# uzh-rpg/dagr

Measured on AMD Instinct MI355X. Metric: events_per_sec, higher is better.
Workload: dtype f32; 1 GPU; dagr-s + --use_image --img_net resnet50, 640x480 synthetic S-uniform, B=8 windows/step x 100000 events (50 ms each), r=7, K=16, events->graph->GNN(+image fusion)->decoded head outputs->confidence mask + NMS (device); image_branch=in-line, engines=3

## Files before the change

dagr_amd/engine.py:

```python
import contextlib
import ctypes
import gc
import types

import numpy as np
import torch

from . import _lib
from .graph.ev_graph import WindowGraphBuilder

FUSED_PASSES_MAX_NODES = 1600

L0_WIDTHS = (8, 16, 32)


def _l0_block(c):
    cm = max(b for b in (0,) + L0_WIDTHS if b <= c)
    return cm, c - cm


def _f32(v):
    return float(torch.as_tensor(v, dtype=torch.float32))


# ... 16 lines not shown
    with torch.cuda.graph(graph):
        gc.disable()
        try:
            yield
        finally:
            if was_enabled:
                gc.enable()

class _ConvPack:

    def __init__(self, cin, cskip, Wm, bias, relu):
        self.K, self.N = Wm.shape
        self.ldw = (self.N + 7) // 8 * 8
        if self.ldw != self.N:
            Wm = torch.cat([Wm, torch.zeros((self.K, self.ldw - self.N), dtype=Wm.dtype, device=Wm.device)], 1)
        self.cin, self.cskip, self.Wm, self.bias, self.relu = cin, cskip, Wm.contiguous(), bias.contiguous(), relu
        K16, N16 = (self.K + 15) // 16 * 16, (self.N + 15) // 16 * 16
        Wp = torch.zeros((K16, N16), dtype=Wm.dtype, device=Wm.device)
        Wp[: self.K, : self.N] = Wm[:, : self.N]
        self.Wq = Wp.view(K16 // 16, 4, 4, N16 // 16, 16).permute(3, 0, 2, 4, 1).contiguous()


def _pack_generic(convs, norms, skip=None, relu=True, device="cuda"):
    cols, biases = [], []
    cin = convs[0].in_channels
    for conv, norm in zip(convs, norms):
        W = conv.weight.detach().float()
        root = conv.lin.weight.detach().float()
        cout = W.shape[2]
        if norm is not None:
            scale, shift = _bn_affine(norm)
        else:
            scale, shift = torch.ones(cout, device=W.device), torch.zeros(cout, device=W.device)
        if conv.bias is not None:
            shift = shift + conv.bias.detach().float() * scale
        block = torch.cat([W.reshape(25 * cin, cout), root.t()], 0) * scale.view(1, -1)
        if skip is not None:
            lin, norm_skip = skip
            s_scale, s_shift = _bn_affine(norm_skip)
            block = torch.cat([block, lin.mlp.weight.detach().float().t() * s_scale.view(1, -1)], 0)
            shift = shift + s_shift
        cols.append(block)
        biases.append(shift)
    cskip = skip[0].mlp.in_features if skip is not None else 0
    return _ConvPack(cin, cskip, torch.cat(cols, 1).to(device), torch.cat(biases).to(device), relu)


def _pack_l0(conv, norm, win, skip=None, device="cuda", cols_in=None, cols_skip=None):
    win_x, tx, win_y, ty = win
    W = conv.weight.detach().float()
    cin, cout = W.shape[1], W.shape[2]
    if cout not in L0_WIDTHS:
        raise NotImplementedError(f"the level-0 kernels exist for {', '.join(map(str, L0_WIDTHS))} output channels "
                                  f"(base_width = 0.25, 0.5, 1.0), not {cout}")
    cols_in = list(range(cin)) if cols_in is None else list(cols_in)
    scale, shift = _bn_affine(norm)
    rows = []
    for b in range(ty):
        for a in range(tx):
            rows.append(W[(win_x + a) + 5 * (win_y + b)][cols_in] * scale.view(1, -1))
    rows.append(conv.lin.weight.detach().float().t()[cols_in] * scale.view(1, -1))
    cskip = 0
    if skip is not None:
        lin, norm_skip = skip
        s_scale, s_shift = _bn_affine(norm_skip)
        ws = lin.mlp.weight.detach().float().t()
        if cols_skip is not None:
            ws = ws[list(cols_skip)]
        rows.append(ws * s_scale.view(1, -1))
        shift = shift + s_shift
        cskip = lin.mlp.in_features
    return cin, cskip, torch.cat(rows, 0).contiguous().to(device), shift.contiguous().to(device)


class _Conv1x1Gemm(torch.nn.Module):

    def __init__(self, conv, relu=False):
        super().__init__()
        cout, cin = conv.weight.shape[:2]
        self.stride = conv.stride[0]
        self.relu = relu
        self.register_buffer("wt", conv.weight.detach().reshape(cout, cin).t().contiguous())
        self.register_buffer("b", conv.bias.detach().clone() if conv.bias is not None else torch.zeros(cout, device=conv.weight.device))

    def forward(self, x, residual=None):
        if self.stride != 1:
            x = x[:, :, ::self.stride, ::self.stride]
        B, C, H, W = x.shape
        a = x.permute(0, 2, 3, 1).reshape(-1, C)
        N = self.wt.shape[1]
        r = None if residual is None else residual.permute(0, 2, 3, 1)
        if _LT["ok"] and a.is_cuda and a.dtype == torch.float32 and a.stride(1) == 1 \
                and (r is None or (r.is_contiguous() and tuple(r.shape) == (B, H, W, N))):
            y = torch.empty((a.shape[0], N), dtype=torch.float32, device=a.device)
            ws = _lt_workspace(a.device)
            act = 1 if (self.relu or r is not None) else 0
            rc = _lib.lib().dagr_gemm_epilogue(_lib.ptr(a), a.shape[0], C, a.stride(0), _lib.ptr(self.wt), N,
                                               _lib.ptr(self.b), _lib.ptr(r), N, act, _lib.ptr(y), N, _lib.ptr(ws),
                                               ws.numel(), _lib.cur_stream(a.device))
            if rc == 0:
                return y.view(B, H, W, -1).permute(0, 3, 1, 2)
            _LT["ok"] = False
        if residual is not None:
            y = torch.addmm(self.b, a, self.wt).view(B, H, W, -1).permute(0, 3, 1, 2)
            return _add_relu_(y, residual)
        y = torch._addmm_activation(self.b, a, self.wt) if self.relu else torch.addmm(self.b, a, self.wt)
        return y.view(B, H, W, -1).permute(0, 3, 1, 2)


_LT = {"ok": True, "ws": {}}


def _lt_workspace(device):
    key = str(device)
    if key not in _LT["ws"]:
        _LT["ws"][key] = torch.empty(int(_lib.lib().dagr_gemm_epilogue_workspace_bytes()), dtype=torch.uint8, device=device)
    return _LT["ws"][key]


def _gemmify_1x1(module):
    for name, child in list(module.named_children()):
        if isinstance(child, torch.nn.Conv2d) and child.kernel_size == (1, 1) and child.groups == 1 \
                and child.padding == (0, 0) and child.stride[0] == child.stride[1]:
            setattr(module, name, _Conv1x1Gemm(child))
        else:
            _gemmify_1x1(child)


def _add_relu_(y, z):
    if y.is_cuda and y.dtype == torch.float32 and z.dtype == torch.float32 and y.shape == z.shape \
            and y.stride() == z.stride() and y.data_ptr() % 16 == 0 and z.data_ptr() % 16 == 0 \
            and (y.is_contiguous() or y.is_contiguous(memory_format=torch.channels_last)):
        _lib.check(_lib.lib().dagr_add_relu(_lib.ptr(y), _lib.ptr(z), y.numel(), _lib.cur_stream(y.device)), "add_relu")
        return y
    return torch.relu_(y.add_(z))


def _bias_relu_(y, bias):
    C = y.shape[1]
    if y.is_cuda and y.dtype == torch.float32 and C % 4 == 0 and y.is_contiguous(memory_format=torch.channels_last) \
            and y.data_ptr() % 16 == 0 and bias.data_ptr() % 16 == 0:
        _lib.check(_lib.lib().dagr_bias_relu(_lib.ptr(y), _lib.ptr(bias), y.numel(), C, _lib.cur_stream(y.device)),
                   "bias_relu")
        return y
    return torch.relu_(y.add_(bias.view(1, -1, 1, 1)))


def _baseconv_forward(m, x):
    y = m.conv(x)
    b = m._bias
    C = y.shape[1]
    if y.is_cuda and y.dtype == torch.float32 and C % 4 == 0 and y.is_contiguous(memory_format=torch.channels_last) \
            and y.data_ptr() % 16 == 0 and b.data_ptr() % 16 == 0:
        _lib.check(_lib.lib().dagr_bias_silu(_lib.ptr(y), _lib.ptr(b), y.numel(), C, _lib.cur_stream(y.device)),
                   "bias_silu")
        return y
    return torch.nn.functional.silu(y.add_(b.view(1, -1, 1, 1)), inplace=True)


def _conv_bias_relu(blk, name, x):
    conv = getattr(blk, name)
    b = getattr(blk, "_" + name + "_bias", None)
    out = conv(x)
    if b is not None:
        return _bias_relu_(out, b)
    if getattr(conv, "relu", False):
        return out
    return blk.relu(out)


def _bottleneck_forward(blk, x):
    identity = x if blk.downsample is None else blk.downsample(x)
    out = _conv_bias_relu(blk, "conv1", x)
    out = _conv_bias_relu(blk, "conv2", out)
    if isinstance(blk.conv3, _Conv1x1Gemm):
        return blk.conv3(out, residual=identity)
    return _add_relu_(blk.conv3(out), identity)


def _resnet_features_forward(net, x, emit=None):
    emit = emit or (lambda name, t: None)
    c1 = net.conv1(x)
    emit("conv1", c1)
    mp = net.maxpool
    ok = (c1.is_cuda and c1.dtype == torch.float32 and c1.is_contiguous(memory_format=torch.channels_last)
          and c1.shape[1] % 4 == 0 and mp.kernel_size == 3 and mp.stride == 2 and mp.padding == 1
          and mp.dilation == 1 and not mp.ceil_mode)
    if ok:
        B, C, H, W = c1.shape
        scale, shift = net._stem_affine
        y = torch.empty((B, C, (H - 1) // 2 + 1, (W - 1) // 2 + 1), dtype=c1.dtype, device=c1.device,
                        memory_format=torch.channels_last)
        _lib.check(_lib.lib().dagr_bn_relu_maxpool(_lib.ptr(c1), B, H, W, C, _lib.ptr(scale), _lib.ptr(shift), _lib.ptr(y),
                                                   _lib.cur_stream(c1.device)), "bn_relu_maxpool")
    else:
        y = net.maxpool(net.relu(net.bn1(c1)))
    l1 = net.layer1(y)
    emit("layer1", l1)
    l2 = net.layer2(l1)
    emit("layer2", l2)
    l3 = net.layer3(l2)
    emit("layer3", l3)
    l4 = net.layer4(l3)
    emit("layer4", l4)
    return dict(conv1=c1, layer1=l1, layer2=l2, layer3=l3, layer4=l4)


def _basicblock_forward(blk, x):
    identity = x if blk.downsample is None else blk.downsample(x)
    out = _conv_bias_relu(blk, "conv1", x)
    return _add_relu_(blk.conv2(out), identity)


class StreamState:

    def __init__(self, batch_size, window_us, device):
        self.B, self.window_us, self.device = int(batch_size), int(window_us), torch.device(device)
        self.cap = 0
        self.state = None
        self.status = torch.zeros((1,), dtype=torch.int32, device=self.device)
        self.lane_count = torch.zeros((self.B,), dtype=torch.int32, device=self.device)
        self.image = None
        self._host = torch.zeros((self.B,), dtype=torch.int32).pin_memory()
        self._known = np.zeros((self.B,), np.int64)
        self._since = 0
        self._fresh = True

    def _alloc(self, cap):
        L = _lib.lib()
        nbytes = L.dagr_stream_state_bytes(self.B, cap)
        if nbytes == 0:
            raise RuntimeError(f"dagr_stream_state_bytes({self.B}, {cap}): out of range")
        return torch.empty(nbytes, dtype=torch.uint8, device=self.device)

    def reset(self):
        if self.state is not None:
            _lib.check(_lib.lib().dagr_stream_reset(_lib.ptr(self.state), self.B, self.cap, _lib.cur_stream(self.device)),
                       "stream_reset")
        self.status.zero_()
        self.lane_count.zero_()
        torch.cuda.current_stream(self.device).synchronize()
        self._host.zero_()
        self._known, self._since, self._fresh = np.zeros((self.B,), np.int64), 0, True

    def grow(self, cap):
# ... 432 lines not shown
                                                1 if pack.relu else 0, stream), "spline_conv_fused")
            return
        lda = (pack.K + 3) // 4 * 4
        _lib.check(L.dagr_spline_tap_aggregate(P(lvl.counts), lvl.T, P(lvl.rowptr), P(lvl.col), P(code),
                                               x, ldx, pack.cin, xskip, ldskip, pack.cskip, dom["rx"], dom["ry"],
                                               dom["den_x"], dom["den_y"], P(scratch), lda, stream), "tap_aggregate")
        _lib.check(L.dagr_gemm_bias_act(P(lvl.counts), lvl.T, P(scratch), lda, P(pack.Wm), pack.ldw, P(pack.bias),
                                        out, ldo, pack.K, pack.N, 1 if pack.relu else 0, stream), "gemm")

    def stage_graph(self, pos, batch, feat=None):
        N = int(pos.shape[0])
        self._alloc_events(N)
        self._N = N
        self._pos, self._batch = pos, batch
        self._nbr = (self.nbr_src[:N], self.nbr_code[:N], self.deg[:N])
        inputs = None
        if feat is not None and pos.dtype == torch.float32:
            self._feat_flat = feat.float().reshape(-1).contiguous()
            inputs = _lib.L0Inputs(feat=self._feat_flat.data_ptr(), pos_nodes=self.pos_n.data_ptr(),
                                   batch_nodes=self.batch_n.data_ptr(), x0=self.x0buf.data_ptr(), ldx0=self.x0_ld,
                                   col_feat=self.x0_feat_col, col_pos=self.x0_pos_col)
        self.graph.build(pos, batch, out=self._nbr, n_dev=self.n_dev if self._dev_mode else None, inputs=inputs)
        self._inputs_gathered = inputs is not None
        self._n_rows = N
        self._async_on = False

    def _nptr(self):
        return self.graph.node_count_ptr() if self._dev_mode else None

    def _sample(self, n_ptr, n_max, pos, batch, b64, fmap, out, coff):
        if self._feat_ready is not None:
            ready = self._feat_ready.get(id(fmap))
            if ready is None:
                raise RuntimeError("pipelined window: a sampled feature map has no ready-event (the image branch did not "
                                   "announce it) -- reading it would race with the image stream")
            torch.cuda.current_stream(self.device).wait_event(ready)
        Bf, C, h, w = fmap.shape
        nhwc = fmap.permute(0, 2, 3, 1)
        if not nhwc.is_contiguous():
            nhwc = nhwc.contiguous()
        self._keep.append(nhwc)
        _lib.check(self.L.dagr_sample_features(n_ptr, n_max, _lib.ptr(pos), _lib.ptr(batch), b64, _lib.ptr(nhwc), Bf, h,
                                               w, C, self.W, self.H, _lib.ptr(out), out.shape[1], coff,
                                               _lib.cur_stream(self.device)), "sample_features")

    def _fold_image_branch(self):
        import copy
        from torch.nn.utils.fusion import fuse_conv_bn_eval
        bb, head = self.model.backbone, self.model.head
        net = copy.deepcopy(bb.net).eval()
        cnn = copy.deepcopy(head.cnn_head).eval()

        def fold_block(blk):
            for ci, bi in (("conv1", "bn1"), ("conv2", "bn2"), ("conv3", "bn3")):
                if hasattr(blk, ci):
                    setattr(blk, ci, fuse_conv_bn_eval(getattr(blk, ci), getattr(blk, bi)))
                    setattr(blk, bi, torch.nn.Identity())
            if blk.downsample is not None:
                blk.downsample = torch.nn.Sequential(fuse_conv_bn_eval(blk.downsample[0], blk.downsample[1]))
        for name in ("layer1", "layer2", "layer3", "layer4"):
            for blk in getattr(net.module, name):
                fold_block(blk)
        for m in cnn.modules():
            if hasattr(m, "conv") and hasattr(m, "bn") and isinstance(m.bn, torch.nn.BatchNorm2d):
                m.conv = fuse_conv_bn_eval(m.conv, m.bn)
                m.bn = torch.nn.Identity()
                if isinstance(getattr(m, "act", None), torch.nn.SiLU) and m.conv.bias is not None:
                    m._bias = m.conv.bias.detach().clone().contiguous()
                    m.conv.bias = None
                    m.forward = types.MethodType(_baseconv_forward, m)
        net = net.to(memory_format=torch.channels_last)
        cnn = cnn.to(memory_format=torch.channels_last)
        for blkname in ("layer1", "layer2", "layer3", "layer4"):
            _gemmify_1x1(getattr(net.module, blkname))
            for blk in getattr(net.module, blkname):
                relu_convs = ("conv1", "conv2") if hasattr(blk, "conv3") else ("conv1",)
                for cname in relu_convs:
                    conv = getattr(blk, cname)
                    if isinstance(conv, _Conv1x1Gemm):
                        conv.relu = True
                    elif isinstance(conv, torch.nn.Conv2d) and conv.bias is not None:
                        setattr(blk, "_" + cname + "_bias", conv.bias.detach().clone().contiguous())
                        conv.bias = None
                blk.forward = types.MethodType(_bottleneck_forward if hasattr(blk, "conv3") else _basicblock_forward,
                                               blk)
        bn = net.module.bn1
        scale = (bn.weight.detach().float() / torch.sqrt(bn.running_var.detach().float() + bn.eps)).contiguous()
        shift = (bn.bias.detach().float() - bn.running_mean.detach().float() * scale).contiguous()
        net.module._stem_affine = (scale, shift)
        net.module.forward_features = types.MethodType(_resnet_features_forward, net.module)
        _gemmify_1x1(net.feature_dconv)
        _gemmify_1x1(net.output_dconv)
        self._net_f, self._cnn_f = net, cnn

    def _image_branch(self, image, on_feature=None):
        if self._net_f is None:
            self._fold_image_branch()
        bb, head = types.SimpleNamespace(net=self._net_f), types.SimpleNamespace(cnn_head=self._cnn_f)
        x = image.contiguous(memory_format=torch.channels_last)
        net = self._net_f
        if on_feature is not None:
            feats = [None] * len(net.feature_layers)

            def emit(name, t):
                if name in net.feature_layers:
                    j = net.feature_layers.index(name)
                    feats[j] = net.feature_dconv[j](t) if len(net.feature_dconv) > 0 else t
                    on_feature(j, feats[j])
            d = _resnet_features_forward(net.module, x, emit)
            outs = [d[l] for l in net.output_layers]
            if len(net.output_dconv) > 0:
                outs = [dconv(o) for o, dconv in zip(outs, net.output_dconv)]
        else:
            feats, outs = bb.net(x)
        outs = outs[-self.num_scales:]
        resized = [torch.nn.functional.interpolate(f, o) for f, o in zip(outs, self.out_sizes)]
        return feats, head.cnn_head(resized)

    def stage_image(self, image):
        self._keep = []
        self._img_feats, self._cnn_out = self._image_branch(image)

    def image_async(self, image, stream=None):
        cur = torch.cuda.current_stream(self.device)
        if stream is not None:
            self._img_stream = stream
        if self._img_stream is None:
            self._img_stream = torch.cuda.Stream(self.device)
        s = self._img_stream
        s.wait_stream(cur)
        with torch.cuda.stream(s):
            feats, cnn_out = self._image_branch(image)
            ev = torch.cuda.Event()
            ev.record(s)
        return feats, cnn_out, ev

    def _consume_image_handle(self, handle):
        feats, cnn_out, ev = handle
        cur = torch.cuda.current_stream(self.device)
        cur.wait_event(ev)
        for t in list(feats) + [o for v in cnn_out.values() for o in v]:
            t.record_stream(cur)
        self._keep = []
        self._img_feats, self._cnn_out = feats, cnn_out

    def stage_l0_input(self, feat):
        N = self._N
        x0 = self.x0buf[:N]
        g = self.graph
        if not self._inputs_gathered:
            f = feat.float().reshape(-1).contiguous()
            _lib.check(self.L.dagr_graph_gather_inputs(ctypes.byref(g.desc), _lib.ptr(g.workspace), _lib.ptr(self._pos),
                                                       _lib.ptr(f), N, _lib.ptr(self.pos_n), _lib.ptr(self.batch_n),
                                                       _lib.ptr(x0), self.x0_ld, self.x0_feat_col, self.x0_pos_col,
                                                       _lib.cur_stream(self.device)), "graph_gather_inputs")
        if self.use_image:
            self._sample(self._nptr(), N, self.pos_n, self.batch_n, 0, self._img_feats[0], x0, self.x0_img_col)
        self._x0 = x0

    def _conv_l0(self, pack, x, ldx, xskip, ldskip, out, ldo):
        L, P = self.L, _lib.ptr
        nbr_src, nbr_code, deg = self._nbr
        cin, cskip, w, s = pack
        d0 = self.dom[0]
        wx, tx, wy, ty = self.win0
        stream = _lib.cur_stream(self.device)
        if self.l0_tiles:
            cm, ce = self._l0_blocks[cin]
            _lib.check(L.dagr_spline_conv_l0_tiles_w(self.cout0, cm, ce, cskip, wx, tx, wy, ty, d0["rx"], d0["ry"],
                                                     d0["den_x"], d0["den_y"], self._N, self.graph.K, P(nbr_src), P(nbr_code),
                                                     P(deg), x, ldx, xskip, ldskip, P(w), P(s), 1, out, ldo, self._nptr(),
                                                     stream), "conv_l0_tiles")
        else:
            _lib.check(L.dagr_spline_conv_l0(cin, cskip, self.ntaps0, self._N, self.graph.K, self.ncodes0, P(nbr_src),
                                             P(nbr_code), P(deg), x, ldx, xskip, ldskip, P(self.tab0), P(w), P(s), 1,
                                             out, ldo, stream), "conv_l0")
# ... 581 lines not shown
```

include/dagr_hip.h:

```cpp
#ifndef DAGR_HIP_H
#define DAGR_HIP_H

#include <stddef.h>
#include <stdint.h>

#ifdef __cplusplus
extern "C" {
#endif

typedef enum {
    DAGR_OK = 0,
    DAGR_ERR_INVALID_ARG = -1,
    DAGR_ERR_HIP = -2,
    DAGR_ERR_WORKSPACE = -3,
    DAGR_ERR_UNSUPPORTED = -4
} dagr_status;

const char *dagr_last_error(void);
int dagr_version(void);
int dagr_device_count(void);

int dagr_format_events(const int16_t *xy , const int32_t *t , const int8_t *p ,
                       int64_t N, int32_t width, int32_t height, int32_t time_window,
                       float *pos_out , float *feat_out , void *stream);
// ... 216 lines not shown
int dagr_spline_conv_fused_pool(const int32_t *n_nodes_ptr, int32_t n_nodes_max, const int32_t *rowptr,
                                const int32_t *col, const int32_t *code, const float *x, int32_t ldx, int32_t cin,
                                const float *xskip, int32_t ldskip, int32_t cskip, int32_t rx, int32_t ry,
                                float den_x, float den_y, const float *Wq, const float *bias, float *C,
                                int32_t ldc, int32_t N, int32_t relu, const dagr_pool_desc *pdesc, void *pool_ws,
                                const float *pos, const int32_t *batch, int32_t *cluster_scratch, void *stream);
int dagr_pool_csr(const dagr_pool_desc *desc, void *pool_ws, const int32_t *n_ptr, int32_t n_max, const float *x,
                  int32_t ldx, const float *pos, const int32_t *batch, const int32_t *rowptr, const int32_t *col,
                  int32_t *cluster_scratch , float *x_out, int32_t ldo, int32_t xoff, float *pos_out,
                  int32_t *batch_out, int32_t *n_out, int32_t *rowptr_out, int32_t *col_out, int32_t *code_out,
                  int32_t *e_out, int32_t e_cap, void *stream);
int dagr_pool_recode(const int32_t *n_ptr, int32_t n_max, const int32_t *rowptr, const int32_t *col, const float *pos,
                     float two_max, float r00, float r02, float r11, float r12, int32_t rx, int32_t ry,
                     int32_t *code_out, int32_t e_cap, int32_t *status, void *stream);
int dagr_pool_status(const dagr_pool_desc *desc, void *pool_ws, int32_t *flags_host, void *stream);
const int32_t *dagr_pool_status_ptr(const dagr_pool_desc *desc, void *pool_ws);
int dagr_pool_counters(const dagr_pool_desc *desc, void *pool_ws, int32_t *out8_host, void *stream);

int dagr_to_dense(const int32_t *n_ptr, int32_t n_max, const float *x, int32_t ldx, int32_t channels,
                  const float *pos, const int32_t *batch, float vx, float vy, int32_t batch_size,
                  int32_t Hc, int32_t Wc, int32_t *winner_scratch, float *dense, int32_t *status, void *stream);

int dagr_pool_argmax(const int32_t *cluster, int32_t n, const float *x, int32_t ldx, int32_t channels,
                     const float *x_pooled, int32_t ldp, int32_t n_clusters, int32_t *arg, void *stream);
int dagr_pool_grad(const int32_t *cluster, int32_t n, int32_t channels, int32_t aggr, const int32_t *arg,
                   const int32_t *count, const float *grad_pooled, int32_t ldg, float *grad_x, int32_t ldgx,
                   void *stream);
int dagr_to_dense_grad(int32_t n, int32_t channels, const float *pos, const int32_t *batch, float vx, float vy,
                       int32_t batch_size, int32_t Hc, int32_t Wc, const float *grad_dense,
                       float *grad_x, int32_t ldgx, void *stream);

int dagr_add_relu(float *y, const float *z, int64_t n, void *stream);
int dagr_bias_relu(float *y_nhwc, const float *bias, int64_t n, int32_t C, void *stream);
int dagr_bias_silu(float *y_nhwc, const float *bias, int64_t n, int32_t C, void *stream);
int dagr_bn_relu_maxpool(const float *x_nhwc, int32_t B, int32_t H, int32_t W, int32_t C, const float *scale,
                         const float *shift, float *y_nhwc, void *stream);

int dagr_sample_features(const int32_t *n_ptr, int32_t n_max, const float *pos, const void *batch,
                         int32_t batch_is_int64, const float *feat_nhwc, int32_t B, int32_t h, int32_t w, int32_t C,
                         int32_t width, int32_t height, float *out, int32_t ldo, int32_t coff, void *stream);

int dagr_nms_batched(const float *boxes, const float *scores, const int32_t *cls, const uint8_t *valid,
                     int32_t B, int32_t A, float iou_threshold, float class_offset,
                     int32_t *order_out, int32_t *keep_out, int32_t *n_keep, void *stream);

typedef struct dagr_head_scale {
    const int32_t *n_ptr; int32_t n_max;
    const float *pred; int32_t ld;
    const float *pos; const int32_t *batch;
    float vx, vy, stride; int32_t Hc, Wc;
    const float *cnn[3]; int32_t cnn_stride[3][4];
    float *dense;
} dagr_head_scale;
int dagr_heads_finish(const dagr_head_scale *scale0, const dagr_head_scale *scale1, int32_t batch_size, int32_t channels,
                      float *out, int32_t *status, void *stream);
int dagr_heads_finish_detect(const dagr_head_scale *scale0, const dagr_head_scale *scale1, int32_t batch_size,
                             int32_t channels, float *out, int32_t *status, float conf_threshold, float iou_threshold,
                             float class_offset, float *det, int32_t *n_keep, void *stream);
int dagr_decode_heads(const float *dense0, int32_t H0, int32_t W0, float stride0, const float *dense1, int32_t H1,
                      int32_t W1, float stride1, int32_t B, int32_t channels, float *out, void *stream);

int dagr_postprocess(const float *pred, int32_t B, int32_t A, int32_t num_classes, float conf_threshold,
                     float iou_threshold, float class_offset, float *det, int32_t *n_keep, void *stream);

int dagr_masked_lin(const int64_t *indices, const float *x_in, float *x_out, const float *weight, const float *bias,
                    int32_t add, int64_t K, int32_t Cin, int32_t Cout, void *stream);
int dagr_masked_lin_no_bias(const int64_t *indices, const float *x_in, float *x_out, const float *weight, int32_t add,
                            int64_t K, int32_t Cin, int32_t Cout, void *stream);
int dagr_masked_isdiff(int64_t *indices, const float *x_old, const float *x_new, float atol, float rtol, int64_t K,
                       int32_t C, void *stream);
int dagr_masked_inplace_BN(const int64_t *indices, const float *x, float *x_out, const float *running_mean,
                           const float *running_var, const float *weight, const float *bias, float eps, int64_t K,
                           int32_t C, void *stream);

int dagr_downsample_events(const int32_t *order, const int32_t *run_cell, const int32_t *run_end, int32_t n_runs,
                           const int8_t *polarity, int32_t fx, int32_t fy, float *change_map, uint8_t *keep,
                           void *stream);

size_t dagr_gemm_epilogue_workspace_bytes(void);
int dagr_gemm_epilogue(const float *A, int64_t M, int32_t K, int64_t lda, const float *Wt, int32_t N, const float *bias,
                       const float *R, int64_t ldr, int32_t act, float *D, int64_t ldd, void *workspace,
                       size_t workspace_bytes, void *stream);

enum { DAGR_FLOPS_ZERO = 0, DAGR_FLOPS_CONV = 1, DAGR_FLOPS_LINEAR = 2, DAGR_FLOPS_POOL = 3, DAGR_FLOPS_CARTESIAN = 4 };
typedef struct dagr_flops_module {
    int32_t kind, level, cin, cout, root, bias;
} dagr_flops_module;
int dagr_async_flops(const int32_t *deg, int32_t n_events, const int32_t *counts1, const int32_t *counts2,
                     const int32_t *counts3, const int32_t *counts4, const dagr_flops_module *mods, int32_t n_mods,
                     int64_t *out, void *stream);

size_t dagr_viz_workspace_bytes(int32_t F, int32_t H, int32_t W);
int dagr_viz_render(const uint8_t *images, int32_t n_images, int32_t H, int32_t W, const int32_t *frame_image, int32_t F,
                    const int32_t *ev_x, const int32_t *ev_y, const int8_t *ev_p, const int32_t *ev_ptr, int32_t n_events,
                    const double *alpha, const int32_t *boxes, const int32_t *box_ptr, int32_t n_boxes, int32_t linewidth,
                    const uint8_t *colors, int32_t n_colors, uint8_t *out, int32_t *status, void *workspace,
                    size_t workspace_bytes, void *stream);

typedef struct dagr_aug_params {
    int32_t flip, crop_on;
    int32_t crop_lo[2], crop_hi[2];
    float zoom;
    int32_t move[2];
} dagr_aug_params;
size_t dagr_augment_workspace_bytes(int64_t N);
int dagr_augment_events(const dagr_aug_params *params, int32_t B, int32_t W, int32_t H, const void *pos, int32_t pos_width,
                        const void *t, int32_t t_width, const void *p, int32_t p_width, const int32_t *sample_ptr, int64_t N,
                        int16_t *out_pos, void *out_t, void *out_p, int64_t *out_batch, int32_t *out_ptr,
                        int32_t *status, void *workspace, size_t workspace_bytes, void *stream);
int dagr_augment_status(const int32_t *status, void *stream);
int dagr_augment_frames(const dagr_aug_params *params, int32_t B, int32_t C, int32_t H, int32_t W, int32_t elem_bytes,
                        int32_t reference_crop, const void *in, void *out, void *stream);
int dagr_augment_boxes(const dagr_aug_params *params, int32_t B, int32_t W, int32_t H, const float *boxes,
                       const int64_t *box_batch, int32_t M, int32_t ld, float *out, void *stream);

#define DAGR_COCO_MAX_GT 256
#define DAGR_COCO_MAX_DT 4096
#define DAGR_COCO_MAX_DETS 100
void dagr_coco_match_bounds(int32_t *max_gt, int32_t *max_dt, int32_t *max_dets);
int dagr_coco_match(const double *gt_xywh, const double *dt_xywh, const double *dt_score, const int64_t *jobs,
                    const double *area_rng, const double *iou_thrs, int32_t n_thr, int32_t max_dets, int64_t n_jobs,
                    int64_t n_gt, int64_t n_dt, int32_t max_gt_per_job, int32_t max_dt_per_job, int64_t n_out,
                    int64_t n_gign, int32_t *order, uint8_t *dtm, uint8_t *dt_ign, uint8_t *g_ign, int32_t *status,
                    void *stream);

#define DAGR_COCO_ACC_TILE 1024
#define DAGR_COCO_ACC_MAX_REC 128
int32_t dagr_coco_accumulate_tile(void);
size_t dagr_coco_accumulate_workspace_bytes(int32_t n_thr, int64_t n_cols);
int dagr_coco_accumulate(const uint8_t *dtm, const uint8_t *dt_ign, const int32_t *perm, const int64_t *group_ptr,
                         const int64_t *group_ngt, const double *rec_thrs, int32_t n_rec, double eps, int32_t n_thr,
                         int32_t n_groups, int64_t n_cols, void *workspace, size_t workspace_bytes, double *precision,
                         int32_t *status, void *stream);

int dagr_spiral_offsets(int32_t n, int32_t *dx_host, int32_t *dy_host);

#ifdef __cplusplus
}
#endif
#endif
```

Before: 143.8 million events/s.

## Route ResNet 1x1 and 3x3 convs through split-bf16 MFMA GEMM kernels

Adds a HIP GEMM kernel that splits FP32 operands into three bf16 parts and accumulates six MFMA cross products, emulating FP32 precision on the bf16 matrix units. The kernel has an implicit-im2col 3x3 mode and a strided 1x1 mode with fused bias, residual and ReLU epilogues. Weights are packed once at fold time, and size heuristics select the new path for the ResNet50 image-branch convolutions. The aim is higher matrix throughput than the FP32 library GEMM and conv paths, at the cost of extra operand splitting work and accuracy that is close to, but not exactly, FP32.

```diff
diff --git a/dagr_amd/csrc/gemm_split_bf16.hip b/dagr_amd/csrc/gemm_split_bf16.hip
--- /dev/null
+++ b/dagr_amd/csrc/gemm_split_bf16.hip
@@ -0,0 +1,334 @@
+#include <algorithm>
+
+#include "common.hpp"
+
+namespace dagr {
+namespace {
+
+constexpr int kKT = 32;
+constexpr int kBN = 128;
+constexpr int kPitch = 40;
+
+typedef __bf16 bf16x8 __attribute__((ext_vector_type(8)));
+typedef float f32x4 __attribute__((ext_vector_type(4)));
+typedef unsigned u32x4 __attribute__((ext_vector_type(4)));
+typedef unsigned u32x2 __attribute__((ext_vector_type(2)));
+
+struct Geo {
+    int mode;
+    int H, W, C, s, Ho, Wo;
+};
+
+struct Args {
+    const float *A;
+    const unsigned short *Wp;
+    const float *bias, *R;
+    float *D;
+    int64_t M, lda, ldr, ldd;
+    int K, N, Npad, act, n_tiles_n, n_blocks;
+    Geo g;
+};
+
+__device__ __forceinline__ unsigned short bf16_bits(__bf16 v) { return __builtin_bit_cast(unsigned short, v); }
+
+__device__ __forceinline__ void split3(float a, unsigned short &p1, unsigned short &p2, unsigned short &p3) {
+    const __bf16 b1 = (__bf16)a;
+    const float r1 = a - (float)b1;
+    const __bf16 b2 = (__bf16)r1;
+    const float r2 = r1 - (float)b2;
+    const __bf16 b3 = (__bf16)r2;
+    p1 = bf16_bits(b1);
+    p2 = bf16_bits(b2);
+    p3 = bf16_bits(b3);
+}
+
+__global__ __launch_bounds__(256) void k_split_pack(const float *__restrict__ Wt, int K, int N, int Npad,
+                                                    unsigned short *__restrict__ out) {
+    const int64_t total = (int64_t)K * Npad;
+    for (int64_t i = (int64_t)blockIdx.x * blockDim.x + threadIdx.x; i < total; i += (int64_t)gridDim.x * blockDim.x) {
+        const int k = (int)(i / Npad), n = (int)(i - (int64_t)k * Npad);
+        unsigned short p[3] = {0, 0, 0};
+        if (n < N) split3(Wt[(int64_t)k * N + n], p[0], p[1], p[2]);
+        const int kt = k / kKT, kk = k - kt * kKT;
+#pragma unroll
+        for (int q = 0; q < 3; q++) out[(((int64_t)kt * 3 + q) * Npad + n) * kKT + kk] = p[q];
+    }
+}
+
+template <int MI, int MODE>
+__global__ __launch_bounds__(256, 3) void k_gemm_split(const Args a) {
+    constexpr int BM = 32 * MI;
+    __shared__ __attribute__((aligned(16))) unsigned short lds[3 * (BM + kBN) * kPitch];
+    unsigned short *const ldsA = lds;
+    unsigned short *const ldsW = lds + 3 * BM * kPitch;
+
+    const int orig = blockIdx.x, xcd = orig & 7, q8 = a.n_blocks >> 3, r8 = a.n_blocks & 7;
+    const int lid = (xcd < r8 ? xcd * (q8 + 1) : r8 * (q8 + 1) + (xcd - r8) * q8) + (orig >> 3);
+    const int nt = lid % a.n_tiles_n, mt = lid / a.n_tiles_n;
+    const int64_t m0 = (int64_t)mt * BM;
+    const int n0 = nt * kBN;
+
+    const int t = threadIdx.x, lane = t & 63, wave = t >> 6;
+    const int wm = wave >> 1, wn = wave & 1;
+
+    const int r0 = t >> 3, c4 = t & 7;
+    int64_t rowoff[MODE == 1 ? MI : 1];
+    int ryx[MODE == 2 ? MI : 1];
+    const int64_t mrow0 = m0 + r0;
+    rowoff[0] = (mrow0 < a.M ? mrow0 : 0) * a.lda;
+    ryx[0] = 0;
+#pragma unroll
+    for (int i = 0; i < MI; i++) {
+        const int64_t m = mrow0 + 32 * i;
+        const int64_t mm = m < a.M ? m : 0;
+        if (MODE == 1) {
+            const int64_t b = mm / ((int64_t)a.g.Ho * a.g.Wo);
+            const int rem = (int)(mm - b * (int64_t)a.g.Ho * a.g.Wo);
+            const int yo = rem / a.g.Wo, xo = rem - yo * a.g.Wo;
+            rowoff[MODE == 1 ? i : 0] = ((b * a.g.H + (int64_t)yo * a.g.s) * a.g.W + (int64_t)xo * a.g.s) * a.lda;
+        } else if (MODE == 2) {
+            ryx[MODE == 2 ? i : 0] = (int)((mm / a.g.W) % a.g.H) << 16 | (int)(mm % a.g.W);
+        }
+    }
+
+    f32x4 ra[MI];
+    u32x4 rw[6];
+    unsigned okmask = 0;
+    const u32x4 *const wbase = reinterpret_cast<const u32x4 *>(a.Wp) + (int64_t)n0 * 4 + t;
+
+    auto gload = [&](int kt) {
+        const int k0 = kt * kKT;
+        int c0 = k0, dy = 0, dx = 0;
+        int64_t toff = 0;
+        if (MODE == 2) {
+            const int tap = k0 / a.g.C;
+            c0 = k0 - tap * a.g.C;
+            dy = tap / 3 - 1;
+            dx = tap - (tap / 3) * 3 - 1;
+            toff = (int64_t)(dy * a.g.W + dx) * a.lda;
+        }
+        okmask = 0;
+#pragma unroll
+        for (int i = 0; i < MI; i++) {
+            bool ok = mrow0 + 32 * i < a.M;
+            if (MODE == 2) {
+                const int yx = ryx[MODE == 2 ? i : 0];
+                ok = ok && (unsigned)((yx >> 16) + dy) < (unsigned)a.g.H && (unsigned)((yx & 0xffff) + dx) < (unsigned)a.g.W;
+            }
+            const int64_t off = MODE == 1 ? rowoff[MODE == 1 ? i : 0] : rowoff[0] + (int64_t)(32 * i) * a.lda;
+            const float *p = ok ? a.A + off + toff + c0 + c4 * 4 : a.A;
+            ra[i] = *reinterpret_cast<const f32x4 *>(p);
+            okmask |= (ok ? 1u : 0u) << i;
+        }
+        const u32x4 *wp = wbase + (int64_t)kt * 3 * a.Npad * 4;
+#pragma unroll
+        for (int p = 0; p < 3; p++) {
+            rw[2 * p] = wp[(int64_t)p * a.Npad * 4];
+            rw[2 * p + 1] = wp[(int64_t)p * a.Npad * 4 + 256];
+        }
+    };
+
+    auto lwrite = [&]() {
+#pragma unroll
+        for (int i = 0; i < MI; i++) {
+            const bool ok = (okmask >> i) & 1u;
+            const f32x4 v = ok ? ra[i] : f32x4{0.f, 0.f, 0.f, 0.f};
+            unsigned short p[3][4];
+#pragma unroll
+            for (int e = 0; e < 4; e++) split3(v[e], p[0][e], p[1][e], p[2][e]);
+#pragma unroll
+            for (int q = 0; q < 3; q++) {
+                const u32x2 u = {(unsigned)p[q][0] | ((unsigned)p[q][1] << 16), (unsigned)p[q][2] | ((unsigned)p[q][3] << 16)};
+                *reinterpret_cast<u32x2 *>(ldsA + (q * BM + r0 + 32 * i) * kPitch + c4 * 4) = u;
+            }
+        }
+#pragma unroll
+        for (int p = 0; p < 3; p++)
+#pragma unroll
+            for (int j = 0; j < 2; j++) {
+                const int c = t + 256 * j;
+                *reinterpret_cast<u32x4 *>(ldsW + (p * kBN + (c >> 2)) * kPitch + (c & 3) * 8) = rw[2 * p + j];
+            }
+    };
+
+    f32x4 acc[MI][4];
+#pragma unroll
+    for (int mi = 0; mi < MI; mi++)
+#pragma unroll
+        for (int ni = 0; ni < 4; ni++) acc[mi][ni] = f32x4{0.f, 0.f, 0.f, 0.f};
+
+    const int frag = (lane & 15) * kPitch + (lane >> 4) * 8;
+    const unsigned short *const fragA = ldsA + (wm * 16 * MI) * kPitch + frag;
+    const unsigned short *const fragW = ldsW + (wn * 64) * kPitch + frag;
+
+    const int n_kt = a.K / kKT;
+    gload(0);
+    lwrite();
+    __syncthreads();
+    for (int kt = 0; kt < n_kt; kt++) {
+        const bool more = kt + 1 < n_kt;
+        if (more) gload(kt + 1);
+        bf16x8 bw[3][4];
+#pragma unroll
+        for (int p = 0; p < 3; p++)
+#pragma unroll
+            for (int ni = 0; ni < 4; ni++)
+                bw[p][ni] = *reinterpret_cast<const bf16x8 *>(fragW + (p * kBN + ni * 16) * kPitch);
+        const f32x4 zero = {0.f, 0.f, 0.f, 0.f};
+#pragma unroll
+        for (int mi = 0; mi < MI; mi++) {
+            bf16x8 av[3];
+#pragma unroll
+            for (int p = 0; p < 3; p++) av[p] = *reinterpret_cast<const bf16x8 *>(fragA + (p * BM + mi * 16) * kPitch);
+            f32x4 ts[4];
+#pragma unroll
+            for (int ni = 0; ni < 4; ni++) ts[ni] = __builtin_amdgcn_mfma_f32_16x16x32_bf16(bw[2][ni], av[0], zero, 0, 0, 0);
+#pragma unroll
+            for (int ni = 0; ni < 4; ni++) ts[ni] = __builtin_amdgcn_mfma_f32_16x16x32_bf16(bw[0][ni], av[2], ts[ni], 0, 0, 0);
+#pragma unroll
+            for (int ni = 0; ni < 4; ni++) ts[ni] = __builtin_amdgcn_mfma_f32_16x16x32_bf16(bw[1][ni], av[1], ts[ni], 0, 0, 0);
+#pragma unroll
+            for (int ni = 0; ni < 4; ni++) ts[ni] = __builtin_amdgcn_mfma_f32_16x16x32_bf16(bw[1][ni], av[0], ts[ni], 0, 0, 0);
+#pragma unroll
+            for (int ni = 0; ni < 4; ni++) ts[ni] = __builtin_amdgcn_mfma_f32_16x16x32_bf16(bw[0][ni], av[1], ts[ni], 0, 0, 0);
+#pragma unroll
+            for (int ni = 0; ni < 4; ni++) ts[ni] = __builtin_amdgcn_mfma_f32_16x16x32_bf16(bw[0][ni], av[0], ts[ni], 0, 0, 0);
+#pragma unroll
+            for (int ni = 0; ni < 4; ni++) acc[mi][ni] += ts[ni];
+            __builtin_amdgcn_sched_barrier(0);
+        }
+        __syncthreads();
+        if (more) {
+            lwrite();
+            __syncthreads();
+        }
+    }
+
+#pragma unroll
+    for (int mi = 0; mi < MI; mi++) {
+        const int64_t m = m0 + wm * 16 * MI + mi * 16 + (lane & 15);
+        if (m >= a.M) continue;
+#pragma unroll
+        for (int ni = 0; ni < 4; ni++) {
+            const int n = n0 + wn * 64 + ni * 16 + (lane >> 4) * 4;
+            if (n >= a.N) continue;
+            f32x4 v = acc[mi][ni];
+            if (a.bias) {
+                const float4 b = *reinterpret_cast<const float4 *>(a.bias + n);
+                v += f32x4{b.x, b.y, b.z, b.w};
+            }
+            if (a.R) {
+                const float4 r = *reinterpret_cast<const float4 *>(a.R + m * a.ldr + n);
+                v += f32x4{r.x, r.y, r.z, r.w};
+            }
+            if (a.act) v = f32x4{fmaxf(v[0], 0.f), fmaxf(v[1], 0.f), fmaxf(v[2], 0.f), fmaxf(v[3], 0.f)};
+            *reinterpret_cast<float4 *>(a.D + m * a.ldd + n) = make_float4(v[0], v[1], v[2], v[3]);
+        }
+    }
+}
+
+inline bool aligned16(const void *p) { return ((uintptr_t)p & 15) == 0; }
+
+template <int MODE>
+int launch(Args &a, int tile, hipStream_t stream) {
+    if (tile == 0) tile = ceil_div(a.M, 64) * a.n_tiles_n >= 2 * (int64_t)device_cu_count() ? 1 : 2;
+    const int bm = tile == 1 ? 64 : 32;
+    const int64_t blocks = ceil_div(a.M, bm) * a.n_tiles_n;
+    DAGR_CHECK_ARG(blocks < ((int64_t)1 << 31), "too many tiles");
+    a.n_blocks = (int)blocks;
+    if (tile == 1)
+        k_gemm_split<2, MODE><<<(unsigned)blocks, 256, 0, stream>>>(a);
+    else
+        k_gemm_split<1, MODE><<<(unsigned)blocks, 256, 0, stream>>>(a);
+    DAGR_CHECK_LAUNCH();
+    return DAGR_OK;
+}
+
+inline int unsupported(const char *fn, const char *what) {
+    set_error(std::string(fn) + ": " + what);
+    return DAGR_ERR_UNSUPPORTED;
+}
+
+}
+}
+
+using namespace dagr;
+
+extern "C" size_t dagr_gemm_split_bf16_packed_bytes(int32_t K, int32_t N) {
+    if (K < kKT || K % kKT != 0 || N < 16 || N % 16 != 0) return 0;
+    return (size_t)K * 3 * align_up((size_t)N, kBN) * sizeof(unsigned short);
+}
+
+extern "C" int dagr_gemm_split_bf16_pack(const float *Wt, int32_t K, int32_t N, void *packed, size_t packed_bytes,
+                                         void *stream) {
+    DAGR_CHECK_ARG(K >= 1 && N >= 1, "bad sizes");
+    if (K % kKT != 0) return unsupported(__func__, "K is not a multiple of the K-tile (32)");
+    if (N % 16 != 0) return unsupported(__func__, "N is not a multiple of 16");
+    DAGR_CHECK_ARG(Wt && packed, "NULL pointer");
+    DAGR_CHECK_ARG(aligned16(packed), "packed is not 16-byte aligned");
+    DAGR_CHECK_ARG(packed_bytes >= dagr_gemm_split_bf16_packed_bytes(K, N), "packed buffer too small");
+    const int Npad = (int)align_up((size_t)N, kBN);
+    const int64_t blocks = std::min<int64_t>(ceil_div((int64_t)K * Npad, 256), 256 * 16);
+    k_split_pack<<<(unsigned)blocks, 256, 0, (hipStream_t)stream>>>(Wt, K, N, Npad, (unsigned short *)packed);
+    DAGR_CHECK_LAUNCH();
+    return DAGR_OK;
+}
+
+namespace {
+int check_common(const char *fn, const float *A, int64_t M, int32_t K, int64_t lda, const void *packed, int32_t N,
+                 const float *bias, const float *R, int64_t ldr, int32_t act, float *D, int64_t ldd, int32_t tile, bool &done) {
+    done = true;
+#define SPLIT_CHECK(cond, msg)                                     \
+    do {                                                           \
+        if (!(cond)) {                                             \
+            set_error(std::string(fn) + ": " + (msg));             \
+            return DAGR_ERR_INVALID_ARG;                           \
+        }                                                          \
+    } while (0)
+    SPLIT_CHECK(M >= 0 && K >= 1 && N >= 1 && ldd >= N && (!R || ldr >= N) && (act == 0 || act == 1) && tile >= 0 && tile <= 2,
+                "bad sizes");
+    if (K % kKT != 0) return unsupported(fn, "K (C of a 3x3) is not a multiple of the K-tile (32)");
+    if (N % 16 != 0) return unsupported(fn, "N is not a multiple of 16");
+    if (M == 0) return DAGR_OK;
+    SPLIT_CHECK(A && packed && D, "NULL pointer");
+    SPLIT_CHECK((const float *)D != A, "D aliases A");
+    SPLIT_CHECK((const float *)D != R, "D aliases R");
+    SPLIT_CHECK(lda % 4 == 0 && ldd % 4 == 0 && (!R || ldr % 4 == 0), "row strides must be multiples of 4 floats");
+    SPLIT_CHECK(aligned16(A) && aligned16(packed) && aligned16(D) && aligned16(bias) && aligned16(R),
+                "pointers must be 16-byte aligned");
+#undef SPLIT_CHECK
+    done = false;
+    return DAGR_OK;
+}
+}
+
+extern "C" int dagr_gemm_split_bf16(const float *A, int64_t M, int32_t K, int64_t lda, const void *packed, int32_t N,
+                                    const float *bias, const float *R, int64_t ldr, int32_t act, float *D, int64_t ldd,
+                                    int32_t B, int32_t H, int32_t W, int32_t stride, int32_t tile, void *stream) {
+    bool done;
+    const int rc = check_common(__func__, A, M, K, lda, packed, N, bias, R, ldr, act, D, ldd, tile, done);
+    if (done) return rc;
+    DAGR_CHECK_ARG(lda >= K && stride >= 1, "bad sizes");
+    Args a{A, (const unsigned short *)packed, bias, R, D, M, lda, R ? ldr : 0, ldd, K, N, (int)align_up((size_t)N, kBN), act,
+           (int)ceil_div(N, kBN), 0, Geo{0, 0, 0, K, 1, 0, 0}};
+    if (stride == 1) return launch<0>(a, tile, (hipStream_t)stream);
+    DAGR_CHECK_ARG(B >= 1 && H >= 1 && W >= 1, "bad image sizes");
+    const int Ho = (H - 1) / stride + 1, Wo = (W - 1) / stride + 1;
+    DAGR_CHECK_ARG(M == (int64_t)B * Ho * Wo, "M is not B * ceil(H / stride) * ceil(W / stride)");
+    a.g = Geo{1, H, W, K, stride, Ho, Wo};
+    return launch<1>(a, tile, (hipStream_t)stream);
+}
+
+extern "C" int dagr_conv3x3_split_bf16(const float *X, int32_t B, int32_t H, int32_t W, int32_t C, int64_t ldx,
+                                       const void *packed, int32_t N, const float *bias, const float *R, int64_t ldr,
+                                       int32_t act, float *D, int64_t ldd, int32_t tile, void *stream) {
+    DAGR_CHECK_ARG(B >= 0 && H >= 1 && W >= 1 && C >= 1 && ldx >= C, "bad sizes");
+    const int64_t M = (int64_t)B * H * W;
+    bool done;
+    const int rc = check_common(__func__, X, M, C, ldx, packed, N, bias, R, ldr, act, D, ldd, tile, done);
+    if (done) return rc;
+    DAGR_CHECK_ARG((int64_t)C * 9 < ((int64_t)1 << 31), "C too large");
+    Args a{X, (const unsigned short *)packed, bias, R, D, M, ldx, R ? ldr : 0, ldd, 9 * C, N, (int)align_up((size_t)N, kBN), act,
+           (int)ceil_div(N, kBN), 0, Geo{2, H, W, C, 1, H, W}};
+    return launch<2>(a, tile, (hipStream_t)stream);
+}
diff --git a/dagr_amd/engine.py b/dagr_amd/engine.py
--- a/dagr_amd/engine.py
+++ b/dagr_amd/engine.py
@@ -122,14 +122,22 @@
         self.relu = relu
         self.register_buffer("wt", conv.weight.detach().reshape(cout, cin).t().contiguous())
         self.register_buffer("b", conv.bias.detach().clone() if conv.bias is not None else torch.zeros(cout, device=conv.weight.device))
+        self.planes = None
+        self.path = None
 
     def forward(self, x, residual=None):
+        N = self.wt.shape[1]
+        r = None if residual is None else residual.permute(0, 2, 3, 1)
+        if self.planes is not None:
+            y = _split_conv(x, self.planes, 1, self.stride, N, self.b, r, self.relu or r is not None)
+            if y is not None:
+                self.path = "split"
+                return y
+        self.path = "library"
         if self.stride != 1:
             x = x[:, :, ::self.stride, ::self.stride]
         B, C, H, W = x.shape
         a = x.permute(0, 2, 3, 1).reshape(-1, C)
-        N = self.wt.shape[1]
-        r = None if residual is None else residual.permute(0, 2, 3, 1)
         if _LT["ok"] and a.is_cuda and a.dtype == torch.float32 and a.stride(1) == 1 \
                 and (r is None or (r.is_contiguous() and tuple(r.shape) == (B, H, W, N))):
             y = torch.empty((a.shape[0], N), dtype=torch.float32, device=a.device)
@@ -158,6 +166,51 @@
     return _LT["ws"][key]
 
 
+def _split_min_rows(K, N, taps):
+    if taps == 1:
+        if K < 128 or N < 128 or K > 512:
+            return None
+        if K <= 256:
+            return 512
+        return 8192 if N >= 256 else None
+    if taps == 9 and K == 128 and N == 128:
+        return 32768
+    return None
+
+
+def _split_pack(wt):
+    L = _lib.lib()
+    K, N = wt.shape
+    nbytes = int(L.dagr_gemm_split_bf16_packed_bytes(K, N))
+    if nbytes == 0 or not wt.is_cuda:
+        return None
+    out = torch.empty(nbytes, dtype=torch.uint8, device=wt.device)
+    _lib.check(L.dagr_gemm_split_bf16_pack(_lib.ptr(wt), K, N, _lib.ptr(out), nbytes, _lib.cur_stream(wt.device)),
+               "gemm_split_bf16_pack")
+    return out
+
+
+def _split_conv(x, planes, taps, stride, N, bias, r, relu):
+    B, C, H, W = x.shape
+    Ho, Wo = (H - 1) // stride + 1, (W - 1) // stride + 1
+    M = B * Ho * Wo
+    rows = _split_min_rows(C, N, taps)
+    xn = x.permute(0, 2, 3, 1)
+    if rows is None or M < rows or not (x.is_cuda and x.dtype == torch.float32 and xn.is_contiguous()) \
+            or (r is not None and not (r.is_contiguous() and tuple(r.shape) == (B, Ho, Wo, N))):
+        return None
+    y = torch.empty((B, Ho, Wo, N), dtype=torch.float32, device=x.device)
+    L, st = _lib.lib(), _lib.cur_stream(x.device)
+    if taps == 1:
+        rc = L.dagr_gemm_split_bf16(_lib.ptr(xn), M, C, C, _lib.ptr(planes), N, _lib.ptr(bias), _lib.ptr(r), N, int(relu),
+                                    _lib.ptr(y), N, B, H, W, stride, 0, st)
+    else:
+        rc = L.dagr_conv3x3_split_bf16(_lib.ptr(xn), B, H, W, C, C, _lib.ptr(planes), N, _lib.ptr(bias), _lib.ptr(r), N,
+                                       int(relu), _lib.ptr(y), N, 0, st)
+    _lib.check(rc, "gemm_split_bf16")
+    return y.permute(0, 3, 1, 2)
+
+
 def _gemmify_1x1(module):
     for name, child in list(module.named_children()):
         if isinstance(child, torch.nn.Conv2d) and child.kernel_size == (1, 1) and child.groups == 1 \
@@ -201,6 +254,14 @@
 def _conv_bias_relu(blk, name, x):
     conv = getattr(blk, name)
     b = getattr(blk, "_" + name + "_bias", None)
+    planes = getattr(conv, "_split_planes", None)
+    if planes is not None:
+        out = _split_conv(x, planes, 9, 1, conv.out_channels, b, None, True)
+        if out is not None:
+            conv._split_path = "split"
+            return out
+    if isinstance(conv, torch.nn.Conv2d):
+        conv._split_path = "library"
     out = conv(x)
     if b is not None:
         return _bias_relu_(out, b)
@@ -799,6 +860,14 @@
                     elif isinstance(conv, torch.nn.Conv2d) and conv.bias is not None:
                         setattr(blk, "_" + cname + "_bias", conv.bias.detach().clone().contiguous())
                         conv.bias = None
+                        if conv.kernel_size == (3, 3) and conv.stride == (1, 1) and conv.padding == (1, 1) \
+                                and conv.dilation == (1, 1) and conv.groups == 1 \
+                                and _split_min_rows(conv.in_channels, conv.out_channels, 9) is not None:
+                            conv._split_planes = _split_pack(conv.weight.detach().permute(2, 3, 1, 0).reshape(
+                                9 * conv.in_channels, conv.out_channels).contiguous())
+                for m in blk.modules():
+                    if isinstance(m, _Conv1x1Gemm) and _split_min_rows(m.wt.shape[0], m.wt.shape[1], 1) is not None:
+                        m.planes = _split_pack(m.wt)
                 blk.forward = types.MethodType(_bottleneck_forward if hasattr(blk, "conv3") else _basicblock_forward,
                                                blk)
         bn = net.module.bn1
@@ -809,6 +878,16 @@
         _gemmify_1x1(net.feature_dconv)
         _gemmify_1x1(net.output_dconv)
         self._net_f, self._cnn_f = net, cnn
+
+    def image_branch_paths(self):
+        if self._net_f is None:
+            return {}
+        out = {}
+        for name, m in self._net_f.named_modules():
+            path = m.path if isinstance(m, _Conv1x1Gemm) else getattr(m, "_split_path", None)
+            if path is not None:
+                out[name] = path
+        return out
 
     def _image_branch(self, image, on_feature=None):
         if self._net_f is None:
diff --git a/include/dagr_hip.h b/include/dagr_hip.h
--- a/include/dagr_hip.h
+++ b/include/dagr_hip.h
@@ -322,6 +322,15 @@
                        const float *R, int64_t ldr, int32_t act, float *D, int64_t ldd, void *workspace,
                        size_t workspace_bytes, void *stream);
 
+size_t dagr_gemm_split_bf16_packed_bytes(int32_t K, int32_t N);
+int dagr_gemm_split_bf16_pack(const float *Wt, int32_t K, int32_t N, void *packed, size_t packed_bytes, void *stream);
+int dagr_gemm_split_bf16(const float *A, int64_t M, int32_t K, int64_t lda, const void *packed, int32_t N,
+                         const float *bias, const float *R, int64_t ldr, int32_t act, float *D, int64_t ldd, int32_t B,
+                         int32_t H, int32_t W, int32_t stride, int32_t tile, void *stream);
+int dagr_conv3x3_split_bf16(const float *X, int32_t B, int32_t H, int32_t W, int32_t C, int64_t ldx, const void *packed,
+                            int32_t N, const float *bias, const float *R, int64_t ldr, int32_t act, float *D, int64_t ldd,
+                            int32_t tile, void *stream);
+
 enum { DAGR_FLOPS_ZERO = 0, DAGR_FLOPS_CONV = 1, DAGR_FLOPS_LINEAR = 2, DAGR_FLOPS_POOL = 3, DAGR_FLOPS_CARTESIAN = 4 };
 typedef struct dagr_flops_module {
     int32_t kind, level, cin, cout, root, bias;
```

New measurement: 151.0 million events/s (median of 6 runs). +5.0%, better.
